# HyeonwooNoh/VQA-Transfer-ExternalData

Hardware: AMD Instinct MI355X
Metric: VQA train samples/sec (img+question) at bs512 (higher is better)
Workload: dtype f32

## Files before the change

include/vqa_hot.h:

```cpp
#ifndef VQA_HOT_H
#define VQA_HOT_H

#include <stdint.h>

#ifdef __cplusplus
extern "C" {
#endif

#define VQA_HOT_ABI_VERSION 5

enum {
    VQA_OK = 0,
    VQA_ERR_ARG = -1,
    VQA_ERR_ALIGN = -2,
    VQA_ERR_LAUNCH = -3,
    VQA_ERR_UNSUPPORTED = -4,
    VQA_ERR_WORKSPACE = -5
};

int vqa_hot_version(void);
const char* vqa_hot_error_string(int code);

int vqa_gather_features(const float* table, const int32_t* nbox_table, const int64_t* idx,
                        float* V, int32_t* nb, int B, int R, int D, int64_t N, void* stream);
// ... 116 lines not shown
int vqa_attn_pool_fwd(const float* v, const float* qv, const float* V, const int32_t* nb, const float* w,
                      const float* bias, const uint8_t* keepmask, float keep_prob, float* att, float* pooled,
                      int B, int R, int H, int D, void* stream);
int vqa_attn_pool_bwd(const float* dpooled, const float* v, const float* qv, const float* V, const float* att,
                      const float* w, const uint8_t* keepmask, float keep_prob, float* dv, float* dqv,
                      float* part_dw, float* part_db, int B, int R, int H, int D, void* stream);

int vqa_attn_set_fast(int on);
int vqa_attn_pool_fwd_rep(const float* v, const float* qv, const float* V, const int32_t* nb, const float* w,
                          const float* bias, const uint8_t* keepmask, float keep_prob, float* att, float* pooled,
                          int B, int rep, int R, int H, int D, void* stream);
int vqa_attn_pool_bwd_rep(const float* dpooled, const float* v, const float* qv, const float* V, const float* att,
                          const float* w, const uint8_t* keepmask, float keep_prob, float* dv, float* dqv,
                          float* part_dw, float* part_db, int B, int rep, int R, int H, int D, void* stream);

enum {
    VQA_STAT_LOSS_TRAIN = 0, VQA_STAT_LOSS_REPORT, VQA_STAT_ALL_SCORE, VQA_STAT_EXIST_SCORE,
    VQA_STAT_TEST_SCORE, VQA_STAT_TEST_OBJ_SCORE, VQA_STAT_TEST_ATTR_SCORE, VQA_STAT_TRAIN_EXIST_SCORE,
    VQA_STAT_MAX_EXIST, VQA_STAT_MAX_TRAIN_EXIST, VQA_STAT_TEST_OBJ_MAX, VQA_STAT_TEST_ATTR_MAX,
    VQA_STAT_TEST_MAX, VQA_STAT_TEST_MAX_EXIST, VQA_STAT_MAX_TRAIN, VQA_STAT_COUNT = 16
};
int vqa_loss_fwd(const float* z, const float* target, const float* train_mask, const float* obj_mask,
                 const float* attr_mask, const float* exist_mask, int use_train_mask_in_loss, float inv_batch,
                 float* stats, int32_t* pred, float* dz, int B, int A, void* stream);
int vqa_loss2_fwd(const float* z_fixed, const float* z_tuned, const float* target, const float* train_mask,
                  const float* obj_mask, const float* attr_mask, const float* exist_mask, float inv_batch, float* stats,
                  int32_t* pred, float* dz_fixed, float* dz_tuned, float* z_sum, int sum_mode, int B, int A, void* stream);
int vqa_rowmin_mask_fwd(const float* z, const float* exist_mask, float* z_masked, float* rowmin, int B, int A, void* stream);
int vqa_rowmin_mask_bwd(float* dz, const float* z, const float* rowmin, const float* exist_mask, int B, int A, void* stream);
int vqa_softmax_ce_fwd(const float* z, const int32_t* label, const float* valid, int topk,
// ... 380 lines not shown
```

vqa-transfer-externaldata_amd/_lib.py:

```python
from __future__ import annotations

import ctypes as C
import os

_HERE = os.path.dirname(os.path.abspath(__file__))
_LIB_PATH = os.path.join(_HERE, "libvqahot.so")


class VqaHotError(RuntimeError):
    pass


def lib_path():
    return _LIB_PATH


class Dims(C.Structure):
    _fields_ = [("B", C.c_int32), ("R", C.c_int32), ("D", C.c_int32), ("H", C.c_int32), ("T", C.c_int32),
                ("W", C.c_int32), ("A", C.c_int32), ("Vq", C.c_int32), ("N_img", C.c_int64),
                ("model_type", C.c_int32), ("keep_att", C.c_float), ("keep_joint", C.c_float),
                ("inv_global_batch", C.c_float), ("flags", C.c_int32),
                ("num_marginal", C.c_int32), ("ent_cols", C.c_int32), ("extra_weight", C.c_float),
                ("map_dim", C.c_int32), ("La", C.c_int32)]

# ... 178 lines not shown
    "vqa_colsum3": (_I, [_P, _P, _P, _I, _I, _I, _P, _P, _P, _P, _L, _P]),
    "vqa_colsum_acc": (_I, [_P, _I, _I, _I, _P, _I, _P, _L, _P]),
    "vqa_colsum3_acc": (_I, [_P, _P, _P, _I, _I, _I, _P, _P, _P, _I, _P, _L, _P]),
    "vqa_mul": (_I, [_P, _P, _P, _L, _P]),
    "vqa_mul_bwd": (_I, [_P, _P, _P, _P, _P, _L, _P]),
    "vqa_add_inplace": (_I, [_P, _P, _L, _P]),
    "vqa_gru_gates_fwd": (_I, [_P, _I, _P, _P, _P, _P, _I, _I, _P]),
    "vqa_gru_cand_fwd": (_I, [_P, _I, _P, _P, _P, _I, _P, _P, _I, _I, _P]),
    "vqa_gru_bwd_a": (_I, [_P, _P, _P, _P, _P, _I, _P, _I, _P, _I, _P, _I, _I, _P]),
    "vqa_gru_bwd_b": (_I, [_P, _P, _P, _P, _I, _P, _I, _I, _P]),
    "vqa_attn_set_fast": (_I, [_I]),
    "vqa_attn_pool_fwd": (_I, [_P, _P, _P, _P, _P, _P, _P, _F, _P, _P, _I, _I, _I, _I, _P]),
    "vqa_attn_pool_bwd": (_I, [_P, _P, _P, _P, _P, _P, _P, _F, _P, _P, _P, _P, _I, _I, _I, _I, _P]),
    "vqa_attn_pool_fwd_rep": (_I, [_P, _P, _P, _P, _P, _P, _P, _F, _P, _P, _I, _I, _I, _I, _I, _P]),
    "vqa_attn_pool_bwd_rep": (_I, [_P, _P, _P, _P, _P, _P, _P, _F, _P, _P, _P, _P, _I, _I, _I, _I, _I, _P]),
    "vqa_loss_fwd": (_I, [_P, _P, _P, _P, _P, _P, _I, _F, _P, _P, _P, _I, _I, _P]),
    "vqa_loss2_fwd": (_I, [_P, _P, _P, _P, _P, _P, _P, _F, _P, _P, _P, _P, _P, _I, _I, _I, _P]),
    "vqa_rowmin_mask_fwd": (_I, [_P, _P, _P, _P, _I, _I, _P]),
    "vqa_rowmin_mask_bwd": (_I, [_P, _P, _P, _P, _I, _I, _P]),
    "vqa_report_reduce": (_I, [_P, _I, _P, _P]),
    "vqa_report_key": (C.c_char_p, [_I]),
    "vqa_sumsq": (_I, [_P, _L, _P, _P, _P, _L, _P]),
    "vqa_sumsq_workspace_floats": (_L, [_L]),
    "vqa_clip_adam": (_I, [_P, _P, _P, _P, _L, _P, _F, _F, _F, _F, _F, _P]),
    "vqa_dropout_mask": (_I, [_P, _L, C.c_uint64, C.c_uint64, _F, _P]),
    "vqa_clip_adam_dev": (_I, [_P, _P, _P, _P, _L, _P, _F, _P, _F, _F, _F, _P]),
    "vqa_embed2_fwd": (_I, [_P, _P, _P, _P, _I, _I, _I, _I, _P]),
    "vqa_embed2_bwd": (_I, [_P, _P, _P, _P, _I, _I, _I, _I, _P]),
    "vqa_lstm_step_fwd": (_I, [_P, _P, _P, _P, _I, _P, _P, _I, _I, _P]),
    "vqa_lstm_step_bwd": (_I, [_P, _P, _P, _P, _P, _P, _I, _P, _P, _P, _I, _I, _P]),
# ... 128 lines not shown
```

vqa-transfer-externaldata_amd/csrc/attention.hip:

```cpp
#include "vqa_common.h"

namespace {

constexpr int MAX_R = 1024;

constexpr int FWD_THREADS = 512;
__global__ __launch_bounds__(FWD_THREADS) void attn_pool_fwd_kernel(
    const float* __restrict__ v, const float* __restrict__ qv, const float* __restrict__ V,
    const int32_t* __restrict__ nb, const float* __restrict__ w, const float* __restrict__ bias,
    const uint8_t* __restrict__ keepmask, float inv_keep, float* __restrict__ att_out, float* __restrict__ pooled, int R,
    int H, int D, int rep) {
    extern __shared__ __attribute__((aligned(16))) float lds[];
    float* qw = lds;
    float* s = lds + H;
    const int b = blockIdx.x, lane = threadIdx.x & 63, wave = threadIdx.x >> 6;
    const int mem = b / rep;
    const float* vb = v + (int64_t)mem * R * H;
    const uint8_t* mb = keepmask ? keepmask + (int64_t)b * R * H : nullptr;
    const float* Vb = V + (int64_t)mem * R * D;

    for (int h = threadIdx.x; h < H; h += FWD_THREADS) qw[h] = qv[(int64_t)b * H + h] * w[h];
    __syncthreads();

    const int H4 = H / 4;
// ... 600 lines not shown
        __syncthreads();
        if (half == 1) {
#pragma unroll
            for (int j = 0; j < REP; ++j) reinterpret_cast<f32x4v*>(comb + (size_t)j * H)[hu] = S[j];
        }
        __syncthreads();
        if (half == 0) {
#pragma unroll
            for (int j = 0; j < REP; ++j) {
                const f32x4v o = reinterpret_cast<const f32x4v*>(comb + (size_t)j * H)[hu];
                const f32x4v t = S[j] + o;
                reinterpret_cast<f32x4v*>(dqv + (q0 + j) * H)[hu] = t * ww;
                reinterpret_cast<f32x4v*>(part_dw + (q0 + j) * H)[hu] = t * qj[j];
            }
        }
    }
}

int g_attn_fast = 1;

}

extern "C" int vqa_attn_set_fast(int on) {
    g_attn_fast = on;
    return VQA_OK;
}

extern "C" int vqa_attn_pool_fwd(const float* v, const float* qv, const float* V, const int32_t* nb, const float* w,
                                 const float* bias, const uint8_t* keepmask, float keep_prob, float* att,
                                 float* pooled, int B, int R, int H, int D, void* stream) {
// ... 120 lines not shown
        VQA_CHECK_LAUNCH();
        return VQA_OK;
    }
    if (rep == 1)
        hipLaunchKernelGGL(attn_pool_bwd_kernel<1>, dim3(B), dim3(BWD_THREADS), lds_for(1), st, dpooled, v, qv, V, att, w,
                           keepmask, ik, dv, dqv, part_dw, part_db, R, H, D, rep);
    else if (rep <= 5)
        hipLaunchKernelGGL(attn_pool_bwd_kernel<5>, dim3(B), dim3(BWD_THREADS), lds_for(5), st, dpooled, v, qv, V, att, w,
                           keepmask, ik, dv, dqv, part_dw, part_db, R, H, D, rep);
    else
        hipLaunchKernelGGL(attn_pool_bwd_kernel<8>, dim3(B), dim3(BWD_THREADS), lds_for(8), st, dpooled, v, qv, V, att, w,
                           keepmask, ik, dv, dqv, part_dw, part_db, R, H, D, rep);
    VQA_CHECK_LAUNCH();
    return VQA_OK;
}
```

vqa-transfer-externaldata_amd/csrc/fusion_model.hip:

```cpp
#include <stdlib.h>
#include <string.h>

#include <string>
#include <vector>

#include "vqa_common.h"

namespace {

struct Entry { const char* name; int64_t off; int64_t n; int esz; };

struct Layout {
    std::vector<Entry> e;
    int64_t total = 0;
    int64_t add(const char* name, int64_t n, int esz = 4) {
        const int64_t off = total;
        e.push_back({name, off, n, esz});
        total += ((n * esz + 255) / 256) * 256;
        return off;
    }
    const Entry* find(const char* name) const {
        for (const auto& x : e)
            if (strcmp(x.name, name) == 0) return &x;
        return nullptr;
// ... 81 lines not shown
    }
    L.add("stats", B * VQA_STAT_COUNT);
    L.add("pred", B);
    L.add("report", 16);
    L.add("dlogit", B * A);
    L.add("d_joint2", B * W);
    L.add("d_joint", B * 2 * H); L.add("d_pre_j", B * 2 * H);
    L.add("d_joint_in", B * H);
    L.add("d_pl", B * H); L.add("d_ll", B * H); L.add("d_pre_pl", B * H); L.add("d_pre_ll", B * H);
    L.add("d_pooled", B * Dp);
    L.add("d_h0", B * H); L.add("d_h1", B * H);
    L.add("d_v", B * R * H); L.add("d_pre_v", B * R * H);
    L.add("d_qv", B * H); L.add("d_pre_qv", B * H);
    L.add("part_a", B * 2 * H); L.add("part_b", B * 2 * H); L.add("part_c", B * 2 * H);
    L.add("part_dw", B * H); L.add("part_db", B);
    L.add("dxp", T * B * 3 * H);
    L.add("d_rh", B * H);
    L.add("dx_embed", T * B * W);
    int64_t gw = 0;
    auto g = [&](int tA, int tB, int64_t M, int64_t N, int64_t K) {
        gw = max64(gw, vqa_gemm_workspace_floats(tA, tB, (int)M, (int)N, (int)K, 0));
        if (d.flags & VQA_FLAG_BF16_GEMM) gw = max64(gw, vqa_gemm_bf16_workspace_floats((int)M, (int)N, (int)K, 0));
    };
    g(0, 0, B * R, H, D); g(0, 0, T * B, 2 * H, W); g(0, 0, T * B, H, W); g(0, 0, B, H, H); g(0, 0, B, H, D);
    g(0, 0, B, 2 * H, H); g(0, 0, B, A, 2 * H);
    g(0, 1, B, 2 * H, A); g(1, 0, 2 * H, A, B); g(0, 1, B, H, 2 * H); g(1, 0, H, 2 * H, B); g(0, 1, B, D, H);
    g(1, 0, D, H, B); g(1, 0, H, H, B); g(0, 1, B, H, H); g(1, 0, D, H, B * R); g(1, 0, W, 2 * H, T * B);
    g(1, 0, H, 2 * H, T * B); g(1, 0, W, H, T * B); g(1, 0, H, H, T * B); g(0, 1, T * B, W, 2 * H);
    g(0, 1, T * B, W, H);
    g(0, 0, T * B, 3 * H, W); g(0, 1, T * B, W, 3 * H); g(1, 0, W, 3 * H, T * B);
// ... 6 lines not shown
        g(0, 0, B * T, H, W); g(0, 1, B * T, W, H); g(1, 0, W, H, B * T);
    }
    if (d.model_type == VQA_MODEL_ENT) {
        const int64_t M = d.num_marginal, C = d.ent_cols;
        g(0, 0, B * M, 2 * H, H); g(0, 0, B * M, C, 2 * H); g(0, 1, B * M, 2 * H, C); g(0, 1, B * M, H, 2 * H);
    }
    if (d.model_type == VQA_MODEL_LEGACY_VQA) legacy_vqa_layout(L, d, gw);
    L.add("gemm_ws", max64(gw, 4));
    L.add("gemm_ws1", max64(gw, 4));
    int64_t cw = 0;
    cw = max64(cw, vqa_colsum_workspace_floats((int)B, (int)(2 * H)));
    cw = max64(cw, vqa_colsum_workspace_floats((int)(T * B), (int)(3 * H)));
    cw = max64(cw, vqa_colsum_workspace_floats((int)B, (int)A));
    cw = max64(cw, vqa_colsum_workspace_floats((int)B, (int)W));
    cw = max64(cw, vqa_colsum_workspace_floats((int)(B * T), (int)H));
    if (d.model_type == VQA_MODEL_LEGACY_VQA)
        cw = max64(cw, max64(max64(vqa_colsum_workspace_floats((int)(T * B), (int)(4 * H)), vqa_colsum_workspace_floats((int)(d.La * A), (int)(4 * H))),
                             vqa_colsum_workspace_floats((int)A, 1)));
    L.add("colsum_ws", max64(3 * cw, 4));
    L.add("colsum_ws1", max64(3 * cw, 4));
    L.add("part_a1", B * H); L.add("part_b1", B * H); L.add("part_c1", B * H);
    L.add("sumsq_ws", max64(vqa_sumsq_workspace_floats(T * B * W), 4));
    L.add("sumsq_ws2", max64(vqa_sumsq_workspace_floats(T * B * W), 4));
    return L;
}

#define TRY(x)                      \
    do {                            \
        int rc__ = (x);             \
        if (rc__ != VQA_OK) return rc__; \
// ... 374 lines not shown
    }
    else if (strcmp(name, "condition") == 0) {
        const Entry* h = L.find("hs");
        if (offset_bytes) *offset_bytes = h->off + (int64_t)dims->T * dims->B * dims->H * 4;
        if (n_elems) *n_elems = (int64_t)dims->B * dims->H;
        return VQA_OK;
    }
    const Entry* e = L.find(key);
    if (e == nullptr) return VQA_ERR_ARG;
    if (offset_bytes) *offset_bytes = e->off;
    if (n_elems) *n_elems = e->n;
    return VQA_OK;
}

namespace {
inline bool visual_late_enabled() {
    static const bool v = [] { const char* e = getenv("VQA_HOT_VISUAL_LATE"); return e == nullptr || atoi(e) != 0; }();
    return v;
}
}

namespace {
inline bool gru_ws_on() {
    static const bool v = [] { const char* e = getenv("VQA_HOT_GRU_WS"); return e == nullptr || atoi(e) != 0; }();
    return v;
}
inline bool xcat_enabled() {
    static const bool v = [] { const char* e = getenv("VQA_HOT_XCAT"); return e == nullptr || atoi(e) != 0; }();
    return v;
}
// ... 333 lines not shown
        if (G->q_L_mean.w != nullptr) {
            TRY(gemm(c, 1, 0, H, H, B, h, (int)H, c.f("d_qm"), (int)H, G->q_L_mean.w, (int)H));
            TRY(colsum(c, c.f("d_qm"), B, H, (int)H, G->q_L_mean.b));
        }
        TRY(gemm(c, 0, 1, B, H, H, c.f("d_qm"), (int)H, P->q_L_mean.w, (int)H, dh, (int)H));
        if (full) {
            if (G->q_L_log_sigma_sq.w != nullptr) {
                TRY(gemm(c, 1, 0, H, H, B, h, (int)H, c.f("d_qs"), (int)H, G->q_L_log_sigma_sq.w, (int)H));
                TRY(colsum(c, c.f("d_qs"), B, H, (int)H, G->q_L_log_sigma_sq.b));
            }
            TRY(gemm(c, 0, 1, B, H, H, c.f("d_qs"), (int)H, P->q_L_log_sigma_sq.w, (int)H, dh, (int)H, nullptr, dh, (int)H));
        }
    } else {
    TRY(ll_bwd(mt == VQA_MODEL_BI ? c.f("q_L_ft") : h, dh));
    }
    {
    ProbeScope ps("attn_pool.bwd", c.st);
    TRY(vqa_attn_pool_bwd(c.f("d_pooled"), c.f("v_linear_v"), c.f("q_linear_v"), c.f(mt == VQA_MODEL_ADAPT ? "v_adapt" : "V_ft"),
                          c.f("att_score"), P->score.w, bt->keep_att, dims->keep_att, c.f("d_v"), c.f("d_qv"), c.f("part_dw"),
                          c.f("part_db"), (int)B, (int)R, (int)H, (int)Dp, c.st));
    }
    if (mt == VQA_MODEL_ADAPT) {
        TRY(vqa_outer_rows(c.f("att_score"), c.f("d_pooled"), c.f("d_va"), (int)B, (int)R, (int)H, c.st));
        TRY(fc_ln_relu_bwd(c, c.f("d_va"), c.f("V_ft"), B * R, D, H, P->v_adapt, &G->v_adapt, (int)R, "pre_va", "mean_va",
                           "rstd_va", nullptr, 1.f, "d_pre_va", nullptr, false));
    }
    if (G->score.w != nullptr) {
        ProbeScope ps("attn_pool.bwd", c.st);
        TRY(colsum(c, c.f("part_dw"), B, H, (int)H, G->score.w));
        TRY(colsum(c, c.f("part_db"), B, 1, 1, G->score.b));
    }
    Side& sd = side_stream();
    const bool forked = fork_side(c, sd);
    {
        Ctx cv{*dims, L, c.ws, forked ? sd.s : c.st, forked ? 1 : 0};
        TRY(fc_ln_relu_bwd(cv, cv.f("d_v"), cv.f("V_ft"), B * R, D, H, P->v_linear_v, &G->v_linear_v, (int)R, "pre_v",
                           "mean_v", "rstd_v", nullptr, 1.f, "d_pre_v", nullptr, false));
        if (forked && !join_side_record(sd)) return VQA_ERR_LAUNCH;
    }
    if (mt == VQA_MODEL_BI) {
        TRY(fc_ln_relu_bwd(c, c.f("d_qv"), c.f("pooled_q_v"), B, H, H, P->q_linear_v, &G->q_linear_v, 1, "pre_qv", "mean_qv",
                           "rstd_qv", nullptr, 1.f, "d_pre_qv", c.f("d_pooled_qv"), false));
        TRY(bi_question_bwd_head(c, P, G, bt, dh));
    } else {
    TRY(fc_ln_relu_bwd(c, c.f("d_qv"), h, B, H, H, P->q_linear_v, &G->q_linear_v, 1, "pre_qv", "mean_qv", "rstd_qv",
                       nullptr, 1.f, "d_pre_qv", dh, true));
    }
    if (forked && hipStreamWaitEvent(c.st, sd.join, 0) != hipSuccess) return VQA_ERR_LAUNCH;
    }
// ... 88 lines not shown
```

vqa-transfer-externaldata_amd/csrc/layernorm.hip:

```cpp
#include "vqa_common.h"

namespace {

constexpr float LN_EPS = 1e-12f;

template <int U>
struct Vec;
template <>
struct Vec<4> {
    float v[4];
    __device__ __forceinline__ void load(const float* p) {
        const float4 t = *reinterpret_cast<const float4*>(p);
        v[0] = t.x; v[1] = t.y; v[2] = t.z; v[3] = t.w;
    }
    __device__ __forceinline__ void store(float* p) const {
        *reinterpret_cast<float4*>(p) = make_float4(v[0], v[1], v[2], v[3]);
    }
    __device__ __forceinline__ void load_mask(const uint8_t* p) {
        const uchar4 t = *reinterpret_cast<const uchar4*>(p);
        v[0] = t.x; v[1] = t.y; v[2] = t.z; v[3] = t.w;
    }
};
template <>
struct Vec<1> {
// ... 304 lines not shown
        float cbias[4] = {0.f, 0.f, 0.f, 0.f};
#pragma unroll
        for (int i = 0; i < RPT; ++i) {
            f32x4v o;
#pragma unroll
            for (int j = 0; j < 4; ++j) {
                const float dp = rstd * (d[c][i][j] - m1 - x[c][i][j] * m2);
                o[j] = dp;
                cbias[j] += ok[i] ? dp : 0.f;
            }
            if (ok[i]) o4[(ry + REG_RY * i) * N4 + cx + REG_CUT * c] = o;
        }
        if (part_dbias != nullptr)
            col_reduce_store<4>(buf0, cbias, part_dbias + (int64_t)g * N, cx + REG_CUT * c, N4, cx, ry, REG_CUT, REG_RY);
    }
}

int g_ln_reg = 1;

inline int reg_mode(int U, int rows, int N) {
    if (!g_ln_reg || U != 4) return 0;
    if (N == REG_CUT * 4 && rows == REG_RY * 9) return 1;
    if (N == REG_CUT * 4 && rows >= 2 && rows <= REG_RY * 2) return 2;
    if (N == REG_CUT * 8 && rows >= 2 && rows <= REG_RY * 2) return 3;
    return 0;
}

struct Shape { int U, CUt, RY, threads; };
Shape pick(const void* a, const void* b, const void* c, int rows, int N, bool mask) {
    Shape s;
// ... 297 lines not shown
            hipLaunchKernelGGL((ln_bwd_reg_kernel<rpt, cpt, false, exact>), dim3(G), dim3(REG_CUT * REG_RY), dyn_reg, st,  \
                               dy, pre, mean, rstd, gamma, beta, keepmask, inv_keep, dpre, part_dgamma, part_dbeta,      \
                               part_dbias, rows);                                                                        \
    } while (0)
        if (rm == 1) VQA_LN_BWD_REG(9, 1, true); else if (rm == 2) VQA_LN_BWD_REG(2, 1, false); else VQA_LN_BWD_REG(2, 2, false);
#undef VQA_LN_BWD_REG
    } else if (s.U == 4)
        hipLaunchKernelGGL(ln_relu_bwd_kernel<4>, dim3(G), dim3(s.threads), dyn, st, dy, pre, mean, rstd, gamma, beta,
                           keepmask, inv_keep, dpre, part_dgamma, part_dbeta, part_dbias, rows, N, s.CUt, s.RY, act);
    else
        hipLaunchKernelGGL(ln_relu_bwd_kernel<1>, dim3(G), dim3(s.threads), dyn, st, dy, pre, mean, rstd, gamma, beta,
                           keepmask, inv_keep, dpre, part_dgamma, part_dbeta, part_dbias, rows, N, s.CUt, s.RY, act);
    VQA_CHECK_LAUNCH();
    return VQA_OK;
}
```

vqa-transfer-externaldata_amd/csrc/rowops.hip:

```cpp
#include "vqa_common.h"

namespace {

inline int64_t cdiv(int64_t a, int64_t b) { return (a + b - 1) / b; }
inline int grid_for(int64_t work_items, int cap = 4096) {
    return (int)std::max<int64_t>(1, std::min<int64_t>(cdiv(work_items, 256), cap));
}

__global__ __launch_bounds__(256) void gather_features_kernel(const float* __restrict__ table,
                                                              const int32_t* __restrict__ nbox_table,
                                                              const int64_t* __restrict__ idx, float* __restrict__ V,
                                                              int32_t* __restrict__ nb, int B, int64_t row_floats,
                                                              int64_t N) {
    const int b = blockIdx.x;
    int64_t src = idx[b];
    if (src < 0) src = 0;
    if (src >= N) src = N - 1;
    if (blockIdx.y == 0 && threadIdx.x == 0 && nb != nullptr) nb[b] = nbox_table[src];
    const float* s = table + src * row_floats;
    float* d = V + (int64_t)b * row_floats;
    const int64_t n4 = row_floats / 4;
    for (int64_t i = blockIdx.y * 256 + threadIdx.x; i < n4; i += (int64_t)gridDim.y * 256)
        reinterpret_cast<float4*>(d)[i] = reinterpret_cast<const float4*>(s)[i];
    if (blockIdx.y == 0)
// ... 261 lines not shown
        for (int m = m0 + ry; m < m1; m += 4) s += X[(int64_t)m * ldx + col];
    red[ry][cx] = s;
    __syncthreads();
    if (ry == 0 && col < N) {
        const float v = red[0][cx] + red[1][cx] + red[2][cx] + red[3][cx];
        float* o = out + (int64_t)blockIdx.y * out_stride_rows + col;
        *o = a.acc[blockIdx.z] ? *o + v : v;
    }
}

__global__ __launch_bounds__(256) void colsum3x4_kernel(Colsum3 a, int M, int N, int ldx, int64_t out_stride_rows,
                                                        int rows_per_chunk) {
    __shared__ cs4 red[4][64];
    colsum4_body(a.X[blockIdx.z], a.out[blockIdx.z], M, N, ldx, (int64_t)blockIdx.y * out_stride_rows, rows_per_chunk,
                 a.acc[blockIdx.z], red);
}

__device__ __forceinline__ uint64_t mix64(uint64_t z) {
    z += 0x9E3779B97F4A7C15ull;
    z = (z ^ (z >> 30)) * 0xBF58476D1CE4E5B9ull;
    z = (z ^ (z >> 27)) * 0x94D049BB133111EBull;
    return z ^ (z >> 31);
}
__device__ __forceinline__ unsigned keep_thr(float keep) {
    const float t = keep * 65536.0f;
    return t <= 0.f ? 0u : (t >= 65536.0f ? 65536u : (unsigned)t);
}
__device__ __forceinline__ unsigned keep_bit(uint64_t key, uint64_t pos, unsigned thr) {
    const uint64_t r = mix64(key ^ (pos >> 2));
    return ((unsigned)(r >> (16 * (pos & 3))) & 0xFFFFu) < thr ? 1u : 0u;
// ... 348 lines not shown
        VQA_COLSUM3_LAUNCH(1, a, M, ldx, std::max(M, 1));
        return VQA_OK;
    }
    VQA_REQUIRE(workspace && workspace_floats >= 3 * (int64_t)ch * N, VQA_ERR_WORKSPACE);
    const int rpc = (int)cdiv(M, ch);
    const int ch2 = (int)cdiv(M, rpc);
    const int64_t zs = (int64_t)ch * N;
    Colsum3 p1{{X0, X1, X2}, {workspace, workspace + zs, workspace + 2 * zs}, {0, 0, 0}};
    VQA_COLSUM3_LAUNCH(ch2, p1, M, ldx, rpc);
    Colsum3 p2{{workspace, workspace + zs, workspace + 2 * zs}, {out0, out1, out2}, {a0, a1, a2}};
    VQA_COLSUM3_LAUNCH(1, p2, ch2, N, ch2);
#undef VQA_COLSUM3_LAUNCH
    return VQA_OK;
}

extern "C" int vqa_dropout_mask(uint8_t* out, int64_t n, uint64_t seed, uint64_t offset, float keep_prob,
                                void* stream) {
    VQA_REQUIRE(out && n >= 0, VQA_ERR_ARG);
    if (n == 0) return VQA_OK;
    if (vqa_aligned16(out))
        hipLaunchKernelGGL(dropout_mask_kernel, dim3(grid_for(n / 16 + 1)), dim3(256), 0, (hipStream_t)stream, out, n, seed,
                           offset, keep_prob);
    else
        hipLaunchKernelGGL(dropout_mask_bytes_kernel, dim3(grid_for(n)), dim3(256), 0, (hipStream_t)stream, out, n, seed,
                           offset, keep_prob);
    VQA_CHECK_LAUNCH();
    return VQA_OK;
}
```

vqa-transfer-externaldata_amd/ops.py:

```python
from __future__ import annotations

import ctypes as C

import numpy as np
import torch

from . import _lib


def _p(t):
    return C.c_void_p(t.data_ptr()) if t is not None else None


def _st(t):
    return C.c_void_p(torch.cuda.current_stream(t.device).cuda_stream)


def _f32(*shape, like):
    return torch.empty(*shape, dtype=torch.float32, device=like.device)


def gemm(A, B, transA=False, transB=False, bias=None, addend=None, split_k=0, out=None):
    lib = _lib.load()
    assert A.dtype == torch.float32 and B.dtype == torch.float32 and A.stride(-1) == 1 and B.stride(-1) == 1
# ... 93 lines not shown
                                     _p(pooled), B, R, H, D, _st(v)), "vqa_attn_pool_fwd")
    return att, pooled


def attn_pool_bwd(dpooled, v, qv, V, att, w, keepmask=None, keep_prob=1.0):
    lib = _lib.load()
    B, R, H = v.shape
    D = V.shape[2]
    dv, dqv = torch.empty_like(v), torch.empty_like(qv)
    pdw, pdb = _f32(B, H, like=v), _f32(B, 1, like=v)
    _lib.check(lib.vqa_attn_pool_bwd(_p(dpooled), _p(v), _p(qv), _p(V), _p(att), _p(w), _p(keepmask), keep_prob,
                                     _p(dv), _p(dqv), _p(pdw), _p(pdb), B, R, H, D, _st(v)), "vqa_attn_pool_bwd")
    return dv, dqv, colsum(pdw), colsum(pdb)


def loss_fwd(z, target, masks, use_train_mask=True, inv_batch=None, want_dz=True):
    lib = _lib.load()
    B, A = z.shape
    stats = _f32(B, 16, like=z)
    pred = torch.empty(B, dtype=torch.int32, device=z.device)
    dz = torch.empty_like(z) if want_dz else None
    _lib.check(lib.vqa_loss_fwd(_p(z), _p(target), _p(masks["train"]), _p(masks["obj"]), _p(masks["attr"]),
                                _p(masks["exist"]), int(use_train_mask), inv_batch if inv_batch else 1.0 / B,
                                _p(stats), _p(pred), _p(dz), B, A, _st(z)), "vqa_loss_fwd")
    report = _f32(16, like=z)
    _lib.check(lib.vqa_report_reduce(_p(stats), B, _p(report), _st(z)), "vqa_report_reduce")
    keys = [lib.vqa_report_key(i).decode() for i in range(13)]
    return stats, pred, dz, dict(zip(keys, report[:13].cpu().tolist()))


# ... 201 lines not shown
```

Measured before the change: 159,900.

## Fuse visual attention tail backward into ds, LN-relu-att and combined colsum kernels

Adds a specialized backward path for the visual attention tail (R=36, H=1024, D=2048). It first computes the score gradient ds directly from dpooled and V. It then folds the per-region attention score backward (dqv, dw) into a register-resident LayerNorm+ReLU backward kernel that recomputes the activations instead of materializing d_v. The partial column sums for gamma, beta, bias, score w and score b are reduced in one launch. This is meant to remove the full B*R*H d_v round trip and several kernel launches. It is enabled by default only when the side stream is unavailable, and it gives up overlap of the v-linear backward with other work.

```diff
diff --git a/include/vqa_hot.h b/include/vqa_hot.h
--- a/include/vqa_hot.h
+++ b/include/vqa_hot.h
@@ -154,6 +154,19 @@
                           const float* w, const uint8_t* keepmask, float keep_prob, float* dv, float* dqv,
                           float* part_dw, float* part_db, int B, int rep, int R, int H, int D, void* stream);
 
+int vqa_vtail_supported(int rep, int R, int H, int D);
+int vqa_vtail_set_mode(int mode);
+int vqa_attn_pool_bwd_ds(const float* dpooled, const float* V, const float* att, float* ds, float* part_db, int B, int rep,
+                         int R, int H, int D, void* stream);
+int vqa_ln_relu_att_bwd(const float* ds, const float* qv, const float* w, const uint8_t* keep_att, float keep_prob,
+                        const float* pre, const float* mean, const float* rstd, const float* gamma, const float* beta,
+                        float* dpre, float* part_dgamma, float* part_dbeta, float* part_dbias, float* dqv, float* part_dw,
+                        int B, int rep, int R, int H, int D, void* stream);
+int64_t vqa_colsum_vtail_workspace_floats(int M, int N);
+int vqa_colsum_vtail(const float* X0, const float* X1, const float* X2, const float* X3, const float* Xb, int M, int N,
+                     float* out0, float* out1, float* out2, float* out3, float* outb, float* workspace,
+                     int64_t workspace_floats, void* stream);
+
 enum {
     VQA_STAT_LOSS_TRAIN = 0, VQA_STAT_LOSS_REPORT, VQA_STAT_ALL_SCORE, VQA_STAT_EXIST_SCORE,
     VQA_STAT_TEST_SCORE, VQA_STAT_TEST_OBJ_SCORE, VQA_STAT_TEST_ATTR_SCORE, VQA_STAT_TRAIN_EXIST_SCORE,
diff --git a/vqa-transfer-externaldata_amd/_lib.py b/vqa-transfer-externaldata_amd/_lib.py
--- a/vqa-transfer-externaldata_amd/_lib.py
+++ b/vqa-transfer-externaldata_amd/_lib.py
@@ -216,6 +216,12 @@
     "vqa_attn_pool_bwd": (_I, [_P, _P, _P, _P, _P, _P, _P, _F, _P, _P, _P, _P, _I, _I, _I, _I, _P]),
     "vqa_attn_pool_fwd_rep": (_I, [_P, _P, _P, _P, _P, _P, _P, _F, _P, _P, _I, _I, _I, _I, _I, _P]),
     "vqa_attn_pool_bwd_rep": (_I, [_P, _P, _P, _P, _P, _P, _P, _F, _P, _P, _P, _P, _I, _I, _I, _I, _I, _P]),
+    "vqa_vtail_supported": (_I, [_I, _I, _I, _I]),
+    "vqa_vtail_set_mode": (_I, [_I]),
+    "vqa_attn_pool_bwd_ds": (_I, [_P, _P, _P, _P, _P, _I, _I, _I, _I, _I, _P]),
+    "vqa_ln_relu_att_bwd": (_I, [_P, _P, _P, _P, _F] + [_P] * 11 + [_I, _I, _I, _I, _I, _P]),
+    "vqa_colsum_vtail_workspace_floats": (_L, [_I, _I]),
+    "vqa_colsum_vtail": (_I, [_P] * 5 + [_I, _I] + [_P] * 6 + [_L, _P]),
     "vqa_loss_fwd": (_I, [_P, _P, _P, _P, _P, _P, _I, _F, _P, _P, _P, _I, _I, _P]),
     "vqa_loss2_fwd": (_I, [_P, _P, _P, _P, _P, _P, _P, _F, _P, _P, _P, _P, _P, _I, _I, _I, _P]),
     "vqa_rowmin_mask_fwd": (_I, [_P, _P, _P, _P, _I, _I, _P]),
diff --git a/vqa-transfer-externaldata_amd/csrc/attention.hip b/vqa-transfer-externaldata_amd/csrc/attention.hip
--- a/vqa-transfer-externaldata_amd/csrc/attention.hip
+++ b/vqa-transfer-externaldata_amd/csrc/attention.hip
@@ -638,6 +638,60 @@
                 reinterpret_cast<f32x4v*>(part_dw + (q0 + j) * H)[hu] = t * qj[j];
             }
         }
+    }
+}
+
+__global__ __launch_bounds__(BWD_THREADS) void attn_pool_bwd_ds_kernel(const float* __restrict__ dpooled,
+                                                                       const float* __restrict__ V,
+                                                                       const float* __restrict__ att,
+                                                                       float* __restrict__ ds_out,
+                                                                       float* __restrict__ part_db, int R) {
+    constexpr int D = 2048, D4 = D / 4, DL = D4 / 64, NW = BWD_THREADS / 64;
+    static_assert(D4 == BWD_THREADS, "dpooled is staged with one float4 per thread");
+    __shared__ __attribute__((aligned(16))) float lds[D + 40];
+    float* ds = lds + D;
+    const int mem = blockIdx.x, lane = threadIdx.x & 63, wave = threadIdx.x >> 6;
+    const int64_t q0 = (int64_t)mem;
+    f32x4v* dp4 = reinterpret_cast<f32x4v*>(lds);
+    {
+        const f32x4v* g4 = reinterpret_cast<const f32x4v*>(dpooled + q0 * D);
+        const f32x4v t = g4[threadIdx.x];
+        dp4[threadIdx.x] = t;
+    }
+    __syncthreads();
+    const f32x4v* Vb4 = reinterpret_cast<const f32x4v*>(V + (int64_t)mem * R * D);
+    for (int r0 = wave; r0 < R; r0 += 2 * NW) {
+        const int rb = min(r0 + NW, R - 1);
+        const bool okb = r0 + NW < R;
+        f32x4v xa[DL], xb[DL];
+#pragma unroll
+        for (int k = 0; k < DL; ++k) {
+            xa[k] = Vb4[(int64_t)r0 * D4 + lane + 64 * k];
+            xb[k] = Vb4[(int64_t)rb * D4 + lane + 64 * k];
+        }
+        float a = 0.f, b = 0.f;
+#pragma unroll
+        for (int k = 0; k < DL; ++k) {
+            const f32x4v g = dp4[lane + 64 * k];
+            a += xa[k].x * g.x + xa[k].y * g.y + xa[k].z * g.z + xa[k].w * g.w;
+            b += xb[k].x * g.x + xb[k].y * g.y + xb[k].z * g.z + xb[k].w * g.w;
+        }
+        a = wave_sum(a);
+        b = wave_sum(b);
+        if (lane == 0) {
+            ds[r0] = a;
+            if (okb) ds[rb] = b;
+        }
+    }
+    __syncthreads();
+    if (wave == 0) {
+        const float a = lane < R ? att[q0 * R + lane] : 0.f;
+        const float d = lane < R ? ds[lane] : 0.f;
+        const float dot = wave_sum(a * d);
+        const float g = a * (d - dot);
+        if (lane < R) ds_out[q0 * R + lane] = g;
+        const float tot = wave_sum(g);
+        if (lane == 0) part_db[q0] = tot;
     }
 }
 
@@ -788,3 +842,19 @@
     VQA_CHECK_LAUNCH();
     return VQA_OK;
 }
+
+extern "C" int vqa_vtail_supported(int rep, int R, int H, int D) {
+    return (rep == 1 && R == 36 && H == 1024 && D == 2048) ? 1 : 0;
+}
+
+extern "C" int vqa_attn_pool_bwd_ds(const float* dpooled, const float* V, const float* att, float* ds, float* part_db,
+                                    int B, int rep, int R, int H, int D, void* stream) {
+    VQA_REQUIRE(dpooled && V && att && ds && part_db && B >= 0, VQA_ERR_ARG);
+    VQA_REQUIRE(vqa_vtail_supported(rep, R, H, D), VQA_ERR_UNSUPPORTED);
+    VQA_REQUIRE(vqa_aligned16(dpooled) && vqa_aligned16(V), VQA_ERR_ALIGN);
+    if (B == 0) return VQA_OK;
+    hipLaunchKernelGGL(attn_pool_bwd_ds_kernel, dim3(B), dim3(BWD_THREADS), 0, (hipStream_t)stream, dpooled, V, att, ds,
+                       part_db, R);
+    VQA_CHECK_LAUNCH();
+    return VQA_OK;
+}
diff --git a/vqa-transfer-externaldata_amd/csrc/fusion_model.hip b/vqa-transfer-externaldata_amd/csrc/fusion_model.hip
--- a/vqa-transfer-externaldata_amd/csrc/fusion_model.hip
+++ b/vqa-transfer-externaldata_amd/csrc/fusion_model.hip
@@ -119,6 +119,7 @@
     L.add("d_qv", B * H); L.add("d_pre_qv", B * H);
     L.add("part_a", B * 2 * H); L.add("part_b", B * 2 * H); L.add("part_c", B * 2 * H);
     L.add("part_dw", B * H); L.add("part_db", B);
+    L.add("ds", B * R);
     L.add("dxp", T * B * 3 * H);
     L.add("d_rh", B * H);
     L.add("dx_embed", T * B * W);
@@ -155,6 +156,7 @@
     cw = max64(cw, vqa_colsum_workspace_floats((int)B, (int)A));
     cw = max64(cw, vqa_colsum_workspace_floats((int)B, (int)W));
     cw = max64(cw, vqa_colsum_workspace_floats((int)(B * T), (int)H));
+    cw = max64(cw, (vqa_colsum_vtail_workspace_floats((int)B, (int)H) + 2) / 3);
     if (d.model_type == VQA_MODEL_LEGACY_VQA)
         cw = max64(cw, max64(max64(vqa_colsum_workspace_floats((int)(T * B), (int)(4 * H)), vqa_colsum_workspace_floats((int)(d.La * A), (int)(4 * H))),
                              vqa_colsum_workspace_floats((int)A, 1)));
@@ -559,6 +561,22 @@
 }
 
 namespace {
+int g_vtail_mode = -1;
+inline int vtail_mode() {
+    if (g_vtail_mode < 0) {
+        const char* e = getenv("VQA_HOT_VTAIL");
+        g_vtail_mode = (e != nullptr && atoi(e) == 0) ? 0 : 1;
+    }
+    return g_vtail_mode;
+}
+}
+
+extern "C" int vqa_vtail_set_mode(int mode) {
+    g_vtail_mode = mode < 0 ? -1 : (mode ? 1 : 0);
+    return vtail_mode();
+}
+
+namespace {
 inline bool visual_late_enabled() {
     static const bool v = [] { const char* e = getenv("VQA_HOT_VISUAL_LATE"); return e == nullptr || atoi(e) != 0; }();
     return v;
@@ -922,6 +940,32 @@
     } else {
     TRY(ll_bwd(mt == VQA_MODEL_BI ? c.f("q_L_ft") : h, dh));
     }
+    Side& sd = side_stream();
+    const bool vtail = vtail_mode() != 0 && !sd.ok && mt != VQA_MODEL_ADAPT && vqa_vtail_supported(1, (int)R, (int)H, (int)Dp) == 1 &&
+                       G->v_linear_v.w != nullptr && G->v_linear_v.gamma != nullptr && G->v_linear_v.beta != nullptr &&
+                       G->v_linear_v.b != nullptr && G->score.w != nullptr && G->score.b != nullptr && vqa_aligned16(c.f("d_pooled")) &&
+                       vqa_aligned16(P->score.w) && vqa_aligned16(P->v_linear_v.gamma) && vqa_aligned16(P->v_linear_v.beta) &&
+                       (bt->keep_att == nullptr || (reinterpret_cast<uintptr_t>(bt->keep_att) & 3u) == 0) &&
+                       vqa_aligned16(G->v_linear_v.gamma) && vqa_aligned16(G->v_linear_v.beta) && vqa_aligned16(G->v_linear_v.b) &&
+                       vqa_aligned16(G->score.w);
+    if (vtail) {
+        {
+            ProbeScope ps("attn_pool.bwd", c.st);
+            TRY(vqa_attn_pool_bwd_ds(c.f("d_pooled"), c.f("V_ft"), c.f("att_score"), c.f("ds"), c.f("part_db"), (int)B, 1, (int)R,
+                                     (int)H, (int)D, c.st));
+        }
+        {
+            ProbeScope ps("v_linear_v.ln_bwd", c.st);
+            TRY(vqa_ln_relu_att_bwd(c.f("ds"), c.f("q_linear_v"), P->score.w, bt->keep_att, dims->keep_att, c.f("pre_v"),
+                                    c.f("mean_v"), c.f("rstd_v"), P->v_linear_v.gamma, P->v_linear_v.beta, c.f("d_pre_v"), c.part(0),
+                                    c.part(1), c.part(2), c.f("d_qv"), c.f("part_dw"), (int)B, 1, (int)R, (int)H, (int)D, c.st));
+            TRY(vqa_colsum_vtail(c.part(0), c.part(1), c.part(2), c.f("part_dw"), c.f("part_db"), (int)B, (int)H,
+                                 G->v_linear_v.gamma, G->v_linear_v.beta, G->v_linear_v.b, G->score.w, G->score.b, c.colsum_ws(),
+                                 c.colsum_ws_floats(), c.st));
+        }
+        ProbeScope ps("v_linear_v.dw_gemm", c.st);
+        TRY(gemm(c, 1, 0, D, H, B * R, c.f("V_ft"), (int)D, c.f("d_pre_v"), (int)H, G->v_linear_v.w, (int)H));
+    } else {
     {
     ProbeScope ps("attn_pool.bwd", c.st);
     TRY(vqa_attn_pool_bwd(c.f("d_pooled"), c.f("v_linear_v"), c.f("q_linear_v"), c.f(mt == VQA_MODEL_ADAPT ? "v_adapt" : "V_ft"),
@@ -938,9 +982,9 @@
         TRY(colsum(c, c.f("part_dw"), B, H, (int)H, G->score.w));
         TRY(colsum(c, c.f("part_db"), B, 1, 1, G->score.b));
     }
-    Side& sd = side_stream();
-    const bool forked = fork_side(c, sd);
-    {
+    }
+    const bool forked = !vtail && fork_side(c, sd);
+    if (!vtail) {
         Ctx cv{*dims, L, c.ws, forked ? sd.s : c.st, forked ? 1 : 0};
         TRY(fc_ln_relu_bwd(cv, cv.f("d_v"), cv.f("V_ft"), B * R, D, H, P->v_linear_v, &G->v_linear_v, (int)R, "pre_v",
                            "mean_v", "rstd_v", nullptr, 1.f, "d_pre_v", nullptr, false));
diff --git a/vqa-transfer-externaldata_amd/csrc/layernorm.hip b/vqa-transfer-externaldata_amd/csrc/layernorm.hip
--- a/vqa-transfer-externaldata_amd/csrc/layernorm.hip
+++ b/vqa-transfer-externaldata_amd/csrc/layernorm.hip
@@ -342,6 +342,114 @@
         if (part_dbias != nullptr)
             col_reduce_store<4>(buf0, cbias, part_dbias + (int64_t)g * N, cx + REG_CUT * c, N4, cx, ry, REG_CUT, REG_RY);
     }
+}
+
+__device__ __forceinline__ float mul_rounded(float a, float b) {
+#pragma clang fp contract(off)
+    return a * b;
+}
+template <bool MASK>
+__global__ __launch_bounds__(REG_CUT * REG_RY) void ln_att_bwd_reg_kernel(
+    const float* __restrict__ ds, const float* __restrict__ qv, const float* __restrict__ w,
+    const uint8_t* __restrict__ keep_att, float inv_keep, const float* __restrict__ pre, const float* __restrict__ mean_in,
+    const float* __restrict__ rstd_in, const float* __restrict__ gamma, const float* __restrict__ beta,
+    float* __restrict__ dpre, float* __restrict__ part_dgamma, float* __restrict__ part_dbeta,
+    float* __restrict__ part_dbias, float* __restrict__ dqv, float* __restrict__ part_dw, int rpt) {
+    constexpr int RPT = 9, N4 = REG_CUT, N = N4 * 4, ROWS = REG_RY * RPT;
+    extern __shared__ __attribute__((aligned(16))) float dyn[];
+    __shared__ float red[16];
+    const int g = blockIdx.x, cx = threadIdx.x % REG_CUT, ry = __builtin_amdgcn_readfirstlane(threadIdx.x / REG_CUT);
+    const int64_t base4 = (int64_t)g * ROWS * N4;
+    const f32x4v* p4 = reinterpret_cast<const f32x4v*>(pre) + base4;
+    const unsigned* m4 = MASK ? reinterpret_cast<const unsigned*>(keep_att) + base4 : nullptr;
+    const float invL = 1.f / ((float)ROWS * (float)N);
+    const float mean = mean_in[g], rstd = rstd_in[g];
+    float* buf0 = dyn;
+    float* buf1 = dyn + (size_t)REG_RY * REG_CUT * 4;
+    f32x4v x[RPT], d[RPT];
+    unsigned km[RPT];
+    float dsr[RPT];
+#pragma unroll
+    for (int i = 0; i < RPT; ++i) {
+        const int o = (ry + REG_RY * i) * N4 + cx;
+        x[i] = p4[o];
+        if (MASK) km[i] = m4[o];
+        dsr[i] = ds[(int64_t)g * ROWS + ry + REG_RY * i];
+        d[i] = (f32x4v)(0.f);
+    }
+    const f32x4v ga = reinterpret_cast<const f32x4v*>(gamma)[cx];
+    const f32x4v be = reinterpret_cast<const f32x4v*>(beta)[cx];
+    float xs = 0.f;
+#pragma unroll
+    for (int i = 0; i < RPT; ++i) { xs += x[i].x; xs += x[i].y; xs += x[i].z; xs += x[i].w; }
+    const float xsum = __builtin_bit_cast(float, __builtin_amdgcn_readfirstlane(__builtin_bit_cast(int, block_sum(xs, red))));
+    float s1 = 0.f, s2 = 0.f;
+    {
+        const f32x4v qj = reinterpret_cast<const f32x4v*>(qv + (int64_t)g * N)[cx];
+        const f32x4v ww = reinterpret_cast<const f32x4v*>(w)[cx];
+        float cb[4] = {0.f, 0.f, 0.f, 0.f}, cg[4] = {0.f, 0.f, 0.f, 0.f}, S[4] = {0.f, 0.f, 0.f, 0.f};
+#pragma unroll
+        for (int i = 0; i < RPT; ++i) {
+            if (i < rpt) {
+                f32x4v gv, rv;
+#pragma unroll
+                for (int j = 0; j < 4; ++j) {
+                    const float xh = (x[i][j] - mean) * rstd;
+                    const float ln = xh * ga[j] + be[j];
+                    float gj = dsr[i];
+                    if (MASK) gj *= (float)((km[i] >> (8 * j)) & 0xFFu) * inv_keep;
+                    gv[j] = gj;
+                    rv[j] = fmaxf(__builtin_fmaf(__builtin_fmaf(-xsum, invL, x[i][j]) * rstd, ga[j], be[j]), 0.f);
+                    float gg = 0.f;
+                    gg += gj * qj[j] * ww[j];
+                    const float dln = ln > 0.f ? gg : 0.f;
+                    const float dxh = dln * ga[j];
+                    s1 += dxh; s2 += dxh * xh; cb[j] += dln; cg[j] += dln * xh;
+                    x[i][j] = xh;
+                    d[i][j] = dxh;
+                }
+                f32x4v* xch = reinterpret_cast<f32x4v*>((i & 1) ? buf1 : buf0);
+                if (ry >= 2) {
+                    xch[(ry - 2) * REG_CUT + cx] = gv;
+                    xch[ry * REG_CUT + cx] = rv;
+                } else {
+#pragma unroll
+                    for (int j = 0; j < 4; ++j) S[j] += gv[j] * rv[j];
+                }
+                __syncthreads();
+                if (ry < 2) {
+                    const f32x4v pg = xch[ry * REG_CUT + cx], pr = xch[(ry + 2) * REG_CUT + cx];
+#pragma unroll
+                    for (int j = 0; j < 4; ++j) S[j] += pg[j] * pr[j];
+                }
+            }
+        }
+        col_reduce_store<4>(buf0, cb, part_dbeta + (int64_t)g * N, cx, N4, cx, ry, REG_CUT, REG_RY);
+        col_reduce_store<4>(buf1, cg, part_dgamma + (int64_t)g * N, cx, N4, cx, ry, REG_CUT, REG_RY);
+        if (ry == 1) reinterpret_cast<f32x4v*>(buf0)[cx] = (f32x4v){S[0], S[1], S[2], S[3]};
+        __syncthreads();
+        if (ry == 0) {
+            const f32x4v t = (f32x4v){S[0], S[1], S[2], S[3]} + reinterpret_cast<const f32x4v*>(buf0)[cx];
+            reinterpret_cast<f32x4v*>(dqv + (int64_t)g * N)[cx] = t * ww;
+            reinterpret_cast<f32x4v*>(part_dw + (int64_t)g * N)[cx] = t * qj;
+        }
+    }
+    const float m1 = block_sum(s1, red) * invL;
+    const float m2 = block_sum(s2, red) * invL;
+    f32x4v* o4 = reinterpret_cast<f32x4v*>(dpre) + base4;
+    float cbias[4] = {0.f, 0.f, 0.f, 0.f};
+#pragma unroll
+    for (int i = 0; i < RPT; ++i) {
+        f32x4v o;
+#pragma unroll
+        for (int j = 0; j < 4; ++j) {
+            const float dp = mul_rounded(rstd, d[i][j] - m1 - x[i][j] * m2);
+            o[j] = dp;
+            cbias[j] += dp;
+        }
+        o4[(ry + REG_RY * i) * N4 + cx] = o;
+    }
+    col_reduce_store<4>(buf0, cbias, part_dbias + (int64_t)g * N, cx, N4, cx, ry, REG_CUT, REG_RY);
 }
 
 int g_ln_reg = 1;
@@ -669,3 +777,31 @@
     VQA_CHECK_LAUNCH();
     return VQA_OK;
 }
+
+extern "C" int vqa_ln_relu_att_bwd(const float* ds, const float* qv, const float* w, const uint8_t* keep_att, float keep_prob,
+                                   const float* pre, const float* mean, const float* rstd, const float* gamma,
+                                   const float* beta, float* dpre, float* part_dgamma, float* part_dbeta, float* part_dbias,
+                                   float* dqv, float* part_dw, int B, int rep, int R, int H, int D, void* stream) {
+    VQA_REQUIRE(ds && qv && w && pre && mean && rstd && gamma && beta && dpre && part_dgamma && part_dbeta && part_dbias && dqv &&
+                    part_dw && B >= 0,
+                VQA_ERR_ARG);
+    VQA_REQUIRE(keep_att == nullptr || keep_prob > 0.f, VQA_ERR_ARG);
+    VQA_REQUIRE(vqa_vtail_supported(rep, R, H, D), VQA_ERR_UNSUPPORTED);
+    VQA_REQUIRE(vqa_aligned16(qv) && vqa_aligned16(w) && vqa_aligned16(pre) && vqa_aligned16(gamma) && vqa_aligned16(beta) &&
+                    vqa_aligned16(dpre) && vqa_aligned16(part_dgamma) && vqa_aligned16(part_dbeta) && vqa_aligned16(part_dbias) &&
+                    vqa_aligned16(dqv) && vqa_aligned16(part_dw) &&
+                    (keep_att == nullptr || (reinterpret_cast<uintptr_t>(keep_att) & 3u) == 0),
+                VQA_ERR_ALIGN);
+    if (B == 0) return VQA_OK;
+    const float inv_keep = keep_att ? 1.f / keep_prob : 1.f;
+    const size_t dyn_reg = (size_t)2 * REG_RY * REG_CUT * 4 * sizeof(float);
+    hipStream_t st = (hipStream_t)stream;
+    if (keep_att != nullptr)
+        hipLaunchKernelGGL((ln_att_bwd_reg_kernel<true>), dim3(B), dim3(REG_CUT * REG_RY), dyn_reg, st, ds, qv, w, keep_att,
+                           inv_keep, pre, mean, rstd, gamma, beta, dpre, part_dgamma, part_dbeta, part_dbias, dqv, part_dw, 9);
+    else
+        hipLaunchKernelGGL((ln_att_bwd_reg_kernel<false>), dim3(B), dim3(REG_CUT * REG_RY), dyn_reg, st, ds, qv, w, keep_att,
+                           inv_keep, pre, mean, rstd, gamma, beta, dpre, part_dgamma, part_dbeta, part_dbias, dqv, part_dw, 9);
+    VQA_CHECK_LAUNCH();
+    return VQA_OK;
+}
diff --git a/vqa-transfer-externaldata_amd/csrc/rowops.hip b/vqa-transfer-externaldata_amd/csrc/rowops.hip
--- a/vqa-transfer-externaldata_amd/csrc/rowops.hip
+++ b/vqa-transfer-externaldata_amd/csrc/rowops.hip
@@ -299,6 +299,29 @@
     __shared__ cs4 red[4][64];
     colsum4_body(a.X[blockIdx.z], a.out[blockIdx.z], M, N, ldx, (int64_t)blockIdx.y * out_stride_rows, rows_per_chunk,
                  a.acc[blockIdx.z], red);
+}
+
+struct Colsum5 { const float* X[5]; float* out[5]; };
+__global__ __launch_bounds__(256) void colsum4x4p1_kernel(Colsum5 a, int M, int N, int ldx, int ldb,
+                                                          int64_t out_stride_rows, int rows_per_chunk) {
+    __shared__ cs4 red[4][64];
+    if (blockIdx.z < 4) {
+        colsum4_body(a.X[blockIdx.z], a.out[blockIdx.z], M, N, ldx, (int64_t)blockIdx.y * out_stride_rows, rows_per_chunk,
+                     0, red);
+        return;
+    }
+    if (blockIdx.x != 0) return;
+    const float* __restrict__ X = a.X[4];
+    float* sred = reinterpret_cast<float*>(red);
+    const int cx = threadIdx.x & 63, ry = threadIdx.x >> 6;
+    const int m0 = blockIdx.y * rows_per_chunk, m1 = min(M, m0 + rows_per_chunk);
+    float s = 0.f;
+    if (cx == 0) {
+        for (int m = m0 + ry; m < m1; m += 4) s += X[(int64_t)m * ldb];
+        sred[ry] = s;
+    }
+    __syncthreads();
+    if (threadIdx.x == 0) a.out[4][blockIdx.y] = sred[0] + sred[1] + sred[2] + sred[3];
 }
 
 __device__ __forceinline__ uint64_t mix64(uint64_t z) {
@@ -677,6 +700,42 @@
     return VQA_OK;
 }
 
+extern "C" int64_t vqa_colsum_vtail_workspace_floats(int M, int N) {
+    const int ch = colsum_chunks(std::max(M, 1));
+    return ch > 1 ? (int64_t)ch * (4 * (int64_t)N + 4) : 0;
+}
+
+extern "C" int vqa_colsum_vtail(const float* X0, const float* X1, const float* X2, const float* X3, const float* Xb, int M,
+                                int N, float* out0, float* out1, float* out2, float* out3, float* outb, float* workspace,
+                                int64_t workspace_floats, void* stream) {
+    VQA_REQUIRE(X0 && X1 && X2 && X3 && Xb && out0 && out1 && out2 && out3 && outb && M >= 0 && N > 0, VQA_ERR_ARG);
+    VQA_REQUIRE(N % 4 == 0 && vqa_aligned16(X0) && vqa_aligned16(X1) && vqa_aligned16(X2) && vqa_aligned16(X3) &&
+                    vqa_aligned16(out0) && vqa_aligned16(out1) && vqa_aligned16(out2) && vqa_aligned16(out3) &&
+                    (workspace == nullptr || vqa_aligned16(workspace)),
+                VQA_ERR_ALIGN);
+    hipStream_t st = (hipStream_t)stream;
+    const int ch = colsum_chunks(std::max(M, 1));
+    const int gx = (N / 4 + 63) / 64;
+    Colsum5 a{{X0, X1, X2, X3, Xb}, {out0, out1, out2, out3, outb}};
+    if (ch == 1) {
+        hipLaunchKernelGGL(colsum4x4p1_kernel, dim3(gx, 1, 5), dim3(256), 0, st, a, M, N, N, 1, (int64_t)N, std::max(M, 1));
+        VQA_CHECK_LAUNCH();
+        return VQA_OK;
+    }
+    VQA_REQUIRE(workspace && workspace_floats >= (int64_t)ch * (4 * (int64_t)N + 4), VQA_ERR_WORKSPACE);
+    const int rpc = (int)cdiv(M, ch);
+    const int ch2 = (int)cdiv(M, rpc);
+    const int64_t zs = (int64_t)ch * N;
+    Colsum5 p1{{X0, X1, X2, X3, Xb}, {workspace, workspace + zs, workspace + 2 * zs, workspace + 3 * zs, workspace + 4 * zs}};
+    hipLaunchKernelGGL(colsum4x4p1_kernel, dim3(gx, ch2, 5), dim3(256), 0, st, p1, M, N, N, 1, (int64_t)N, rpc);
+    VQA_CHECK_LAUNCH();
+    Colsum5 p2{{workspace, workspace + zs, workspace + 2 * zs, workspace + 3 * zs, workspace + 4 * zs},
+               {out0, out1, out2, out3, outb}};
+    hipLaunchKernelGGL(colsum4x4p1_kernel, dim3(gx, 1, 5), dim3(256), 0, st, p2, ch2, N, N, 1, (int64_t)N, ch2);
+    VQA_CHECK_LAUNCH();
+    return VQA_OK;
+}
+
 extern "C" int vqa_dropout_mask(uint8_t* out, int64_t n, uint64_t seed, uint64_t offset, float keep_prob,
                                 void* stream) {
     VQA_REQUIRE(out && n >= 0, VQA_ERR_ARG);
diff --git a/vqa-transfer-externaldata_amd/ops.py b/vqa-transfer-externaldata_amd/ops.py
--- a/vqa-transfer-externaldata_amd/ops.py
+++ b/vqa-transfer-externaldata_amd/ops.py
@@ -131,6 +131,36 @@
     return dv, dqv, colsum(pdw), colsum(pdb)
 
 
+def attn_pool_bwd_ds(dpooled, V, att):
+    lib = _lib.load()
+    B, R, D = V.shape
+    ds, pdb = _f32(B, R, like=V), _f32(B, like=V)
+    _lib.check(lib.vqa_attn_pool_bwd_ds(_p(dpooled), _p(V), _p(att), _p(ds), _p(pdb), B, 1, R, 1024, D, _st(V)),
+               "vqa_attn_pool_bwd_ds")
+    return ds, pdb
+
+
+def ln_relu_att_bwd(ds, qv, w, pre, mean, rstd, gamma, beta, keepmask=None, keep_prob=1.0):
+    lib = _lib.load()
+    B, R, H = pre.shape
+    dpre = torch.empty_like(pre)
+    pg, pb, pbias, dqv, pdw = (_f32(B, H, like=pre) for _ in range(5))
+    _lib.check(lib.vqa_ln_relu_att_bwd(_p(ds), _p(qv), _p(w), _p(keepmask), keep_prob, _p(pre), _p(mean), _p(rstd),
+                                       _p(gamma), _p(beta), _p(dpre), _p(pg), _p(pb), _p(pbias), _p(dqv), _p(pdw), B, 1, R,
+                                       H, 2048, _st(pre)), "vqa_ln_relu_att_bwd")
+    return dpre, (pg, pb, pbias), dqv, pdw
+
+
+def colsum_vtail(X0, X1, X2, X3, Xb):
+    lib = _lib.load()
+    M, N = X0.shape
+    outs = [_f32(N, like=X0) for _ in range(4)] + [_f32(1, like=X0)]
+    ws = _f32(max(int(lib.vqa_colsum_vtail_workspace_floats(M, N)), 4), like=X0)
+    _lib.check(lib.vqa_colsum_vtail(_p(X0), _p(X1), _p(X2), _p(X3), _p(Xb), M, N, *[_p(o) for o in outs], _p(ws),
+                                    ws.numel(), _st(X0)), "vqa_colsum_vtail")
+    return outs
+
+
 def loss_fwd(z, target, masks, use_train_mask=True, inv_batch=None, want_dz=True):
     lib = _lib.load()
     B, A = z.shape
```

Result: faster. 161,600 (median of 6 runs) (+1.1%).
